# JeanElsner/practical-multi-view

Measured on AMD Instinct MI355X. Metric: VO frames/sec on 1241x376 KITTI mono @400 tracks, bundle=5, higher is better.
Workload: dtype u8/int32 front-end, f64 back-end

## Files before the change

### practical-multi-view_amd/csrc/backend_ba.hip

```cpp
#include "pmv_ctx.h"
#include <algorithm>
#include "backend.h"
#include "pmv_prof.h"
#include <float.h>

namespace pmv {

typedef double v4d __attribute__((ext_vector_type(4)));

constexpr int BA_T = 512;
constexpr int BA_NW = BA_T / 64;


__device__ inline void angle_axis_rotate(const double a[3], const double q[3], double p[3], double dpdw[9], double Rm[9], bool jac) {
    const double theta2 = a[0] * a[0] + a[1] * a[1] + a[2] * a[2];
    if (theta2 > DBL_EPSILON) {
        const double theta = sqrt(theta2);
        const double ct = cos(theta), st = sin(theta), ti = 1.0 / theta;
        const double w[3] = {a[0] * ti, a[1] * ti, a[2] * ti};
        const double wxq[3] = {w[1] * q[2] - w[2] * q[1], w[2] * q[0] - w[0] * q[2], w[0] * q[1] - w[1] * q[0]};
        const double wq = w[0] * q[0] + w[1] * q[1] + w[2] * q[2];
        const double tmp = wq * (1.0 - ct);
#pragma unroll
        for (int i = 0; i < 3; i++) p[i] = q[i] * ct + wxq[i] * st + w[i] * tmp;
// ... 1103 lines not shown
    gmax_p = wave_max_f64(gmax_p);
    if (lane == 0) red[wid] = gmax_p;
    __syncthreads();
    if (tid == 0) part_gmax[sl] = fmax(fmax(red[0], red[1]), fmax(red[2], red[3]));
    const int eb0 = A.pobs_start[p0], eb1 = A.pobs_start[p1];
    for (int e = eb0 + tid; e < eb1; e += BM_T) {
        const int4 rec = A.erec[e];
        if (rec.w == 2) continue;
        const int c = rec.y, pp = rec.z;
        double w[18], y[18];
        bam_obs_wy(A, Jb, e, rec, sEi + (pp - p0) * 9, w, y);
#pragma unroll
        for (int b = 0; b < 3; b++) {
            const int kr = 3 * pp + b - k0;
            if (kr < 0 || kr >= k1 - k0) continue;
#pragma unroll
            for (int a = 0; a < 6; a++) {
                Wl[(size_t)(6 * c + a) * stride + kr] = w[a * 3 + b];
                Yl[(size_t)(6 * c + a) * stride + kr] = y[a * 3 + b];
            }
        }
    }
    __syncthreads();
    const int tc = A.tiles_c;
    if (wid < A.tiles_r * tc) {
        const int ti = wid / tc, tj = wid - ti * tc;
        const double* pa = Yl + (size_t)(ti * 16 + (lane & 15)) * stride + 4 * (lane >> 4);
        const double* pb = Wl + (size_t)(tj * 16 + (lane & 15)) * stride + 4 * (lane >> 4);
        const v4d acc = schur_tile_mfma(pa, pb, (k1 - k0) / 16);
#pragma unroll
        for (int r = 0; r < 4; r++)
            A.Gpart[((size_t)sl * A.gp_rows + ti * 16 + (lane >> 4) + 4 * r) * ldw + tj * 16 + (lane & 15)] = acc[r];
    }
}

__global__ __launch_bounds__(BM_T) void k_bam_pointgemm(BAArgs A, const BAGState* st_in, BAGState* st_out, const double* part4, int nbp,
                                                        int* chol_flag, double* Ublk, double* rhsblk, double* part_gmax) { BACKEND_PRIO();
    extern __shared__ __attribute__((aligned(16))) double dyn[];
    __shared__ BAGState ss;
    __shared__ double ssc[8];
    const int bid = blockIdx.x;
    if (threadIdx.x == 0) {
        ss = *st_in;
        if (!ss.done) bam_decide(ss, part4, nbp);
        if (bid == 0) *st_out = ss;
    }
    __syncthreads();
    if (bid < A.nc) bam_cam_role(A, ss, bid, Ublk, rhsblk, dyn, ssc);
    else bam_slice_role(A, ss, chol_flag, bid - A.nc, part_gmax, dyn);
}

constexpr int BG_W = 4, BG_H = 2;
__device__ inline void bam_gemm_role(const BAArgs& A, const BAGState* st, int bid, double* sacc ) {
    static_assert(BG_W * 4 * 64 <= BM_NW * 4 * 64, "LDS");
    if (st->done) return;
    const int lane = threadIdx.x & 63, wv = threadIdx.x >> 6, krows = A.krows, ldw = A.ldw;
    const int tc = A.tiles_c;
    const int tile = bid / BG_H, half = bid % BG_H;
    const int ti = tile / tc, tj = tile - ti * tc;
    const int kper = A.kper;
    const int k0 = min(krows, (half * BG_W + wv) * kper), k1 = min(krows, k0 + kper);
    const double* pa = A.Yd + (size_t)(ti * 16 + (lane & 15)) * krows + 4 * (lane >> 4) + k0;
    const double* pb = A.Wd + (size_t)(tj * 16 + (lane & 15)) * krows + 4 * (lane >> 4) + k0;
    const v4d acc = schur_tile_mfma(pa, pb, (k1 - k0) / 16);
#pragma unroll
    for (int r = 0; r < 4; r++) sacc[(wv * 4 + r) * 64 + lane] = acc[r];
    __syncthreads();
    if (wv == 0) {
#pragma unroll
        for (int r = 0; r < 4; r++) {
            double g = sacc[r * 64 + lane];
#pragma unroll
            for (int w = 1; w < BG_W; w++) g += sacc[(w * 4 + r) * 64 + lane];
            A.Gpart[((size_t)half * A.gp_rows + ti * 16 + (lane >> 4) + 4 * r) * ldw + tj * 16 + (lane & 15)] = g;
        }
    }
}

__global__ __launch_bounds__(64 * BG_W) void k_bam_gemm(BAArgs A, const BAGState* st) { BACKEND_PRIO();
    __shared__ double swork[BG_W * 4 * 64];
    bam_gemm_role(A, st, blockIdx.x, swork);
}

__device__ inline const BAGState* bam_solve_role(const BAArgs& A, const BAGState* st_in, BAGState* st_out, bool writer,
                                                 const int* __restrict__ chol_flag, const double* __restrict__ part_cost,
                                                 int nbo, const double* __restrict__ part_gmax, int nbp, const double* __restrict__ Ublk,
                                                 const double* __restrict__ rhsblk, double* __restrict__ candrot, double* candrot_l, int gslices) {
    extern __shared__ __attribute__((aligned(16))) double dyn[];
    __shared__ double red[3 * BM_NW];
    __shared__ BAGState ss;
    __shared__ int sfail;
    const int tid = threadIdx.x, lane = tid & 63, wid = tid >> 6;
    const int tx = tid & 15, ty = tid >> 4;
    unsigned long long t_prev = __builtin_readcyclecounter();
#define SSTAMP(k) do { if (A.stamps && writer && tid == 0) { const unsigned long long t_ = __builtin_readcyclecounter(); A.stamps[k] += t_ - t_prev; t_prev = t_; } } while (0)
#define SPUBLISH() do { if (writer && tid == 0) *st_out = ss; } while (0)
    if (tid == 0) { ss = *st_in; sfail = 0; }
    __syncthreads();
    if (ss.done) { SPUBLISH(); return nullptr; }
    const int nc = A.nc, m = 6 * nc, n = m + 3 * A.np;
    double* S = dyn; double* dg = dyn + (size_t)(m + 1) * m;
    const double* x = A.x + (size_t)ss.cur * n;
    if (ss.need_eval) {
        double g = 0, cs = 0;
        for (int i = tid; i < m; i += BM_T) g = fmax(g, fabs(rhsblk[i] / A.scale[i]));
        for (int i = tid; i < nbp; i += BM_T) g = fmax(g, part_gmax[i]);
        for (int i = tid; i < nbo; i += BM_T) cs += part_cost[i];
        cs = wave_sum_f64(cs);
        g = wave_max_f64(g);
        if (lane == 0) { red[BM_NW + wid] = cs; red[2 * BM_NW + wid] = g; }
        __syncthreads();
        if (tid == 0) {
            if (ss.first) {
                const double c = (red[BM_NW] + red[BM_NW + 1]) + (red[BM_NW + 2] + red[BM_NW + 3]);
                ss.x_cost = c;
                ss.initial_cost = c;
            }
            ss.gmax = fmax(fmax(red[2 * BM_NW], red[2 * BM_NW + 1]), fmax(red[2 * BM_NW + 2], red[2 * BM_NW + 3]));
        }
    }
    if (tid == 0) {
        int term = -1;
        if (ss.iter >= ss.max_iterations) term = 0;
        else if (ss.gmax >= 0 && ss.gmax <= 1e-10) term = 2;
        else if (ss.radius < 1e-32) term = 4;
        if (term >= 0) { ss.done = 1; ss.termination = term; }
        ss.step_valid = 0;
    }
    __syncthreads();
    if (ss.done) { SPUBLISH(); return nullptr; }
    SSTAMP(16);
    {
        const double radius = ss.radius;
        const bool reuse = ss.reuse_diag != 0;
        for (int a = ty; a <= m; a += 16) {
            for (int b = tx; b < m && b <= a; b += 16) {
                double v;
                if (a < m) v = (a / 6 == b / 6) ? Ublk[(a / 6) * 36 + (a % 6) * 6 + (b % 6)] : 0.0;
                else v = rhsblk[b];
                const size_t gi = (a < m) ? (size_t)a * A.ldw + b : (size_t)b * A.ldw + m;
                double g;
                if (gslices) {
                    double hsum[BG_H];
#pragma unroll
                    for (int h = 0; h < BG_H; h++) {
#pragma unroll
                        for (int w = 0; w < BG_W; w++) {
                            const int sl = h * BG_W + w;
                            const double v = sl < gslices ? A.Gpart[(size_t)sl * A.gp_rows * A.ldw + gi] : 0.0;
                            hsum[h] = w == 0 ? v : hsum[h] + v;
                        }
                    }
                    g = hsum[0];
#pragma unroll
                    for (int h = 1; h < BG_H; h++) g += hsum[h];
                } else {
                    g = A.Gpart[gi];
#pragma unroll
                    for (int h = 1; h < BG_H; h++) g += A.Gpart[(size_t)h * A.gp_rows * A.ldw + gi];
                }
                if (a == b) {
                    double d2;
                    if (!reuse) { d2 = fmin(fmax(v, 1e-6), 1e32); if (writer) A.diag[a] = d2; }
                    else d2 = A.diag[a];
                    v += d2 / radius;
                }
                S[(size_t)a * m + b] = v - g;
            }
        }
    }
    __syncthreads();
    if (*chol_flag) { SPUBLISH(); return nullptr; }
    SSTAMP(17);
    for (int jb = 0; jb < nc; jb++) {
        const int j0 = 6 * jb;
        if (tid == 0) {
            double a[21];
#pragma unroll
            for (int i = 0; i < 6; i++) {
#pragma unroll
                for (int k = 0; k <= i; k++) a[i * (i + 1) / 2 + k] = S[(size_t)(j0 + i) * m + j0 + k];
            }
            bool ok = true;
            double r[6];
#pragma unroll
            for (int j = 0; j < 6; j++) {
                const double d = a[j * (j + 1) / 2 + j];
                ok = ok && (d > 0.0);
                r[j] = rsqrt_nr(d);
                a[j * (j + 1) / 2 + j] = d * r[j];
#pragma unroll
                for (int i = j + 1; i < 6; i++) a[i * (i + 1) / 2 + j] *= r[j];
#pragma unroll
                for (int i = j + 1; i < 6; i++) {
#pragma unroll
                    for (int k = j + 1; k <= i; k++) a[i * (i + 1) / 2 + k] -= a[i * (i + 1) / 2 + j] * a[k * (k + 1) / 2 + j];
                }
            }
#pragma unroll
            for (int i = 0; i < 6; i++) {
#pragma unroll
                for (int k = 0; k <= i; k++) S[(size_t)(j0 + i) * m + j0 + k] = a[i * (i + 1) / 2 + k];
                dg[j0 + i] = r[i];
            }
            if (!ok) sfail = 1;
        }
        __syncthreads();
        if (sfail) break;
        {
            const int i = j0 + 6 + tid;
            if (i <= m) {
                double v[6], Lb[15], r[6];
#pragma unroll
                for (int k = 0; k < 6; k++) { v[k] = S[(size_t)i * m + j0 + k]; r[k] = dg[j0 + k]; }
#pragma unroll
                for (int q = 1; q < 6; q++) {
#pragma unroll
                    for (int k = 0; k < q; k++) Lb[q * (q - 1) / 2 + k] = S[(size_t)(j0 + q) * m + j0 + k];
                }
#pragma unroll
                for (int q = 0; q < 6; q++) {
                    double t = v[q];
#pragma unroll
                    for (int k = 0; k < q; k++) t -= v[k] * Lb[q * (q - 1) / 2 + k];
                    v[q] = t * r[q];
                }
#pragma unroll
                for (int k = 0; k < 6; k++) S[(size_t)i * m + j0 + k] = v[k];
            }
        }
        __syncthreads();
        {
            const int r0 = j0 + 6;
            const int nr = m - r0;
            const int total = nr * (nr + 1) / 2 + nr;
            for (int e = tid; e < total; e += BM_T) {
                int ii = (int)((sqrtf(8.0f * (float)e + 1.0f) - 1.0f) * 0.5f);
                while ((ii + 1) * (ii + 2) / 2 <= e) ii++;
                while (ii * (ii + 1) / 2 > e) ii--;
                int kk = e - ii * (ii + 1) / 2;
                if (ii >= nr) { ii = nr; kk = e - nr * (nr + 1) / 2; }
                const double* Li = S + (size_t)(r0 + ii) * m + j0;
                const double* Lk = S + (size_t)(r0 + kk) * m + j0;
                double acc = S[(size_t)(r0 + ii) * m + r0 + kk];
#pragma unroll
                for (int t = 0; t < 6; t++) acc -= Li[t] * Lk[t];
                S[(size_t)(r0 + ii) * m + r0 + kk] = acc;
            }
        }
        __syncthreads();
    }
    if (sfail) { SPUBLISH(); return nullptr; }
    SSTAMP(18);
    if (wid == 0) {
        double* ys = S + (size_t)m * m;
        for (int jb = nc - 1; jb >= 0; jb--) {
            const int j0 = 6 * jb;
            double xb[6], Lb[15], r[6];
#pragma unroll
            for (int q = 0; q < 6; q++) { xb[q] = ys[j0 + q]; r[q] = dg[j0 + q]; }
#pragma unroll
            for (int q = 1; q < 6; q++) {
#pragma unroll
                for (int k = 0; k < q; k++) Lb[q * (q - 1) / 2 + k] = S[(size_t)(j0 + q) * m + j0 + k];
            }
#pragma unroll
            for (int q = 5; q >= 0; q--) {
                double t = xb[q];
#pragma unroll
                for (int k = 5; k > q; k--) t -= Lb[k * (k - 1) / 2 + q] * xb[k];
                xb[q] = t * r[q];
            }
            for (int k = lane; k < j0; k += 64) {
                double acc = ys[k];
#pragma unroll
                for (int t = 5; t >= 0; t--) acc -= S[(size_t)(j0 + t) * m + k] * xb[t];
                ys[k] = acc;
            }
            if (lane < 6) {
                double v = xb[0];
#pragma unroll
                for (int t = 1; t < 6; t++) v = (lane == t) ? xb[t] : v;
                ys[j0 + lane] = v;
            }
            WAVE_SYNC();
        }
        for (int k = lane; k < m; k += 64) { const double v = -ys[k]; if (writer) A.step[k] = v; S[k] = v; }
        WAVE_SYNC();
        SSTAMP(19);
        if (lane < nc) {
            double cx[6];
#pragma unroll
            for (int k = 0; k < 6; k++) cx[k] = x[6 * lane + k] + S[6 * lane + k] * A.scale[6 * lane + k];
            CamRot cr;
            cam_rot_setup(cx, cr);
            const double cv[7] = {cr.ct, cr.st, cr.ti, cr.w0, cr.w1, cr.w2, (double)cr.big};
            if (writer) {
                double* o = candrot + 16 * lane;
#pragma unroll
                for (int k = 0; k < 6; k++) o[k] = cx[k];
#pragma unroll
                for (int k = 0; k < 7; k++) o[6 + k] = cv[k];
            }
            if (candrot_l) {
                double* o = candrot_l + 16 * lane;
#pragma unroll
                for (int k = 0; k < 6; k++) o[k] = cx[k];
#pragma unroll
                for (int k = 0; k < 7; k++) o[6 + k] = cv[k];
            }
        }
        if (lane == 0) ss.step_valid = 1;
        SSTAMP(20);
    }
    __syncthreads();
    SPUBLISH();
    return &ss;
#undef SPUBLISH
#undef SSTAMP
}

__device__ inline void bam_backsub_role(const BAArgs& A, const BAGState* st, const double* step_c, const double* candrot,
                                        double* __restrict__ tmp3, double* __restrict__ part4, int bid) {
    __shared__ double red[4 * BM_NW];
    __shared__ double sP[BM_PB * 6];
    if (st->done || !st->step_valid) return;
    const int tid = threadIdx.x;
    unsigned long long t_prev = __builtin_readcyclecounter();
#define BSTAMP(k) do { if (A.stamps && bid == 0 && tid == 0) { const unsigned long long t_ = __builtin_readcyclecounter(); A.stamps[k] += t_ - t_prev; t_prev = t_; } } while (0)
    const int nc = A.nc, m = 6 * nc, n = m + 3 * A.np;
    const int cur = st->cur;
    const double* x = A.x + (size_t)cur * n;
    double* cand = A.x + (size_t)(cur ^ 1) * n;
    const double* Jb = A.J + (size_t)cur * A.nobs * 18;
    const double* resb = A.res + (size_t)cur * A.nobs * 2;
    double* Jn = A.J + (size_t)(cur ^ 1) * A.nobs * 18;
    double* resn = A.res + (size_t)(cur ^ 1) * A.nobs * 2;
    const bool spec = st->iter + 1 < st->max_iterations;
    const int p0 = bid * BM_PB, p1 = min(A.np, p0 + BM_PB);
    const int eb0 = A.pobs_start[p0], eb1 = A.pobs_start[p1];
    double mc = 0, cc = 0, dn2 = 0, xn2 = 0;
    for (int e = eb0 + tid; e < eb1; e += BM_T) {
        const int4 rec = A.erec[e];
        const int i = rec.x, c = rec.y;
        const double* Jr = Jb + (size_t)i * 18;
        double jy0 = 0, jy1 = 0;
#pragma unroll
        for (int a = 0; a < 6; a++) { const double yc = -step_c[6 * c + a]; jy0 += Jr[a] * yc; jy1 += Jr[6 + a] * yc; }
#pragma unroll
        for (int a = 0; a < 3; a++) tmp3[(size_t)e * 3 + a] = Jr[12 + a] * jy0 + Jr[15 + a] * jy1;
    }
    __syncthreads();
    BSTAMP(10);
    const int p = p0 + tid;
    if (tid < BM_PB && p < p1) {
        double t3[3] = {A.gp[(size_t)p * 3], A.gp[(size_t)p * 3 + 1], A.gp[(size_t)p * 3 + 2]};
        for (int e = A.pobs_start[p]; e < A.pobs_start[p + 1]; e++) {
#pragma unroll
            for (int a = 0; a < 3; a++) t3[a] -= tmp3[(size_t)e * 3 + a];
        }
        const double* Ei = A.Einv + (size_t)p * 9;
#pragma unroll
        for (int a = 0; a < 3; a++) {
            const double sp = -(Ei[a * 3] * t3[0] + Ei[a * 3 + 1] * t3[1] + Ei[a * 3 + 2] * t3[2]);
            A.step[m + 3 * p + a] = sp;
            const double d = sp * A.scale[m + 3 * p + a];
            const double xo = x[m + 3 * p + a];
            xn2 += xo * xo;
            const double xp = xo + d;
            cand[m + 3 * p + a] = xp;
            sP[tid * 6 + a] = sp; sP[tid * 6 + 3 + a] = xp;
            dn2 += d * d;
        }
    }
    __syncthreads();
    BSTAMP(11);
    for (int e = eb0 + tid; e < eb1; e += BM_T) {
        const int4 rec = A.erec[e];
        const int i = rec.x, c = rec.y, pl = rec.z - p0;
        const double* Jr = Jb + (size_t)i * 18;
        double sc[6], sp[3], xp[3];
#pragma unroll
        for (int k = 0; k < 6; k++) sc[k] = step_c[6 * c + k];
#pragma unroll
        for (int k = 0; k < 3; k++) { sp[k] = sP[pl * 6 + k]; xp[k] = sP[pl * 6 + 3 + k]; }
#pragma unroll
        for (int rr = 0; rr < 2; rr++) {
            double mr = 0;
#pragma unroll
            for (int k = 0; k < 6; k++) mr += Jr[rr * 6 + k] * sc[k];
#pragma unroll
            for (int k = 0; k < 3; k++) mr += Jr[12 + rr * 3 + k] * sp[k];
            mc -= mr * (resb[2 * i + rr] + mr / 2.0);
        }
        const double* o = candrot + 16 * c;
        CamRot cr;
        cr.ct = o[6]; cr.st = o[7]; cr.ti = o[8]; cr.w0 = o[9]; cr.w1 = o[10]; cr.w2 = o[11]; cr.big = (int)o[12];
        double r[2], rho0, rho1;
        if (spec) {
            double Jc[12], Jp[6];
            projection_residual_pre(cr, o, xp, A.obs[2 * i], A.obs[2 * i + 1], A.K, r, Jc, Jp, true);
            huber_rho(r[0] * r[0] + r[1] * r[1], A.huber, rho0, rho1);
            const double sr = sqrt(rho1);
            resn[2 * i] = r[0] * sr; resn[2 * i + 1] = r[1] * sr;
            const double* scc = A.scale + 6 * c;
            const double* scp = A.scale + 6 * A.nc + 3 * (pl + p0);
            double* Jo = Jn + (size_t)i * 18;
#pragma unroll
            for (int k = 0; k < 12; k++) Jo[k] = Jc[k] * sr * scc[k % 6];
#pragma unroll
            for (int k = 0; k < 6; k++) Jo[12 + k] = Jp[k] * sr * scp[k % 3];
        } else {
            projection_residual_pre(cr, o, xp, A.obs[2 * i], A.obs[2 * i + 1], A.K, r, nullptr, nullptr, false);
            huber_rho(r[0] * r[0] + r[1] * r[1], A.huber, rho0, rho1);
        }
        cc += 0.5 * rho0;
    }
    BSTAMP(12);
    if (bid == 0) {
        for (int i = tid; i < m; i += BM_T) {
            const double d = step_c[i] * A.scale[i];
            cand[i] = x[i] + d;
            dn2 += d * d;
            xn2 += x[i] * x[i];
        }
    }
    mc = wave_sum_f64(mc); cc = wave_sum_f64(cc); dn2 = wave_sum_f64(dn2); xn2 = wave_sum_f64(xn2);
    if ((tid & 63) == 0) { red[tid >> 6] = mc; red[BM_NW + (tid >> 6)] = cc; red[2 * BM_NW + (tid >> 6)] = dn2; red[3 * BM_NW + (tid >> 6)] = xn2; }
    __syncthreads();
    if (tid == 0) {
        part4[bid * 4] = (red[0] + red[1]) + (red[2] + red[3]);
        part4[bid * 4 + 1] = (red[BM_NW] + red[BM_NW + 1]) + (red[BM_NW + 2] + red[BM_NW + 3]);
        part4[bid * 4 + 2] = (red[2 * BM_NW] + red[2 * BM_NW + 1]) + (red[2 * BM_NW + 2] + red[2 * BM_NW + 3]);
        part4[bid * 4 + 3] = (red[3 * BM_NW] + red[3 * BM_NW + 1]) + (red[3 * BM_NW + 2] + red[3 * BM_NW + 3]);
    }
    BSTAMP(13);
#undef BSTAMP
}

__global__ __launch_bounds__(BM_T) void k_bam_solveback(BAArgs A, const BAGState* st_in, BAGState* st_out, const int* chol_flag,
                                                        const double* part_cost, int nbo, const double* part_gmax, int ngm,
                                                        const double* Ublk, const double* rhsblk, double* candrot, double* tmp3,
                                                        double* part4, int gslices) { BACKEND_PRIO();
    extern __shared__ __attribute__((aligned(16))) double dyn[];
    const int m = 6 * A.nc;
    double* candrot_l = dyn + (size_t)(m + 1) * m + m;
    const BAGState* ss = bam_solve_role(A, st_in, st_out, blockIdx.x == 0, chol_flag, part_cost, nbo, part_gmax, ngm, Ublk, rhsblk, candrot, candrot_l, gslices);
    if (!ss) return;
    bam_backsub_role(A, ss, dyn, candrot_l, tmp3, part4, blockIdx.x);
}

__device__ inline void bam_finish_role(const BAArgs& A, const BAGState* __restrict__ st_in, const double* __restrict__ part4, int nbp) {
    __shared__ BAGState ss;
    if (threadIdx.x == 0) {
        ss = *st_in;
        if (!ss.done) bam_decide(ss, part4, nbp);
    }
    __syncthreads();
    const int n = 6 * A.nc + 3 * A.np;
    const double* x = A.x + (size_t)ss.cur * n;
    double* ocams = A.out ? A.out + BA_SUM_SLOTS : A.cams;
    double* opts = A.out ? A.out + BA_SUM_SLOTS + 6 * A.nc : A.pts;
    double* osum = A.out ? A.out : A.summary;
    for (int i = threadIdx.x; i < 6 * A.nc; i += BM_T) ocams[i] = x[i];
    for (int i = threadIdx.x; i < 3 * A.np; i += BM_T) opts[i] = x[6 * A.nc + i];
    if (threadIdx.x == 0) {
        osum[0] = ss.initial_cost; osum[1] = ss.x_cost; osum[2] = ss.iter; osum[3] = ss.successful;
        osum[4] = ss.termination;
    }
    if (A.out && A.done_seq) {
        __threadfence_system();
        __syncthreads();
        if (threadIdx.x == 0) __hip_atomic_store((unsigned*)(A.out + BA_SUM_DONE), A.done_seq, __ATOMIC_RELEASE, __HIP_MEMORY_SCOPE_SYSTEM);
    }
}

__global__ __launch_bounds__(BM_T) void k_bam_finish(BAArgs A, const BAGState* st_in, const double* part4, int nbp) { BACKEND_PRIO();
    bam_finish_role(A, st_in, part4, nbp);
}

hipError_t launch_ba_multi(hipStream_t s, const BAArgs& A, void* d_state, double* d_part) {
    BAGState* sa = (BAGState*)d_state;
    BAGState* sb = (BAGState*)((char*)d_state + 256);
    int* chol_flags = (int*)((char*)d_state + 512);
    static_assert(sizeof(BAGState) <= 256, "BAGState");
    const int nbo = (A.nobs + BM_T - 1) / BM_T, nbp = (A.np + BM_PB - 1) / BM_PB, m = 6 * A.nc;
    double* part_cost = d_part;
    double* part_gmax = part_cost + nbo;
    double* part4 = part_gmax + nbp + 8;
    double* Ublk = part4 + 4 * nbp;
    double* rhsblk = Ublk + 36 * A.nc;
    double* candrot = rhsblk + 6 * A.nc;
    double* tmp3 = candrot + 16 * A.nc;
    const size_t shm = ((size_t)(m + 1) * m + (size_t)m + (size_t)16 * A.nc) * sizeof(double);
    if (A.max_iterations > BA_MAX_ITERATIONS || shm > 150 * 1024) return hipErrorInvalidValue;
    ProfScope ps(K_BA_LM, s);
    const int tiles = A.tiles_r * A.tiles_c;
    const size_t shm_pg = std::max(bam_slice_lds(A.ldw, A.kper), (size_t)BM_WORK * sizeof(double));
    const bool fused = tiles <= BM_NW && A.kslices <= BG_H * BG_W && shm_pg <= 150 * 1024 && bam_slice_points(A.kper) <= BM_T;
    const int clear_blocks = (int)std::min<size_t>(64, ((size_t)A.krows * A.ldw + 4 * BM_T - 1) / (4 * BM_T));
    { ProfScope p_(K_BAM_EVAL0, s);
    hipLaunchKernelGGL(k_bam_eval0, dim3(nbo + clear_blocks), dim3(BM_T), 0, s, A, sa, chol_flags, part_cost, nbo); }
    for (int it = 0; it < A.max_iterations; it++) {
        int* cf = chol_flags + it;
        if (it == 0) {
            ProfScope p_(K_BAM_CAMPOINT, s);
            hipLaunchKernelGGL(k_bam_campoint, dim3(A.nc), dim3(BM_T), 0, s, A, sa, sa, 0, part4, nbp, cf, A.nc, Ublk, rhsblk, part_gmax);
            hipLaunchKernelGGL(k_bam_campoint, dim3(nbp), dim3(BM_T), 0, s, A, sa, sa, 0, part4, nbp, cf, 0, Ublk, rhsblk, part_gmax);
        } else if (fused) {
            ProfScope p_(K_BAM_POINTGEMM, s);
            hipLaunchKernelGGL(k_bam_pointgemm, dim3(A.nc + A.kslices), dim3(BM_T), shm_pg, s, A, sb, sa, part4, nbp, cf, Ublk, rhsblk, part_gmax);
        } else {
            ProfScope p_(K_BAM_CAMPOINT, s);
            hipLaunchKernelGGL(k_bam_campoint, dim3(A.nc + nbp), dim3(BM_T), 0, s, A, sb, sa, 1, part4, nbp, cf, A.nc, Ublk, rhsblk, part_gmax);
        }
        const bool sliced = fused && it > 0;
        if (!sliced) { ProfScope p_(K_BAM_GEMM, s);
        hipLaunchKernelGGL(k_bam_gemm, dim3(tiles * BG_H), dim3(64 * BG_W), 0, s, A, sa); }
        { ProfScope p_(K_BAM_SOLVEBACK, s);
        hipLaunchKernelGGL(k_bam_solveback, dim3(nbp), dim3(BM_T), shm, s, A, sa, sb, cf, part_cost, nbo, part_gmax, sliced ? A.kslices : nbp, Ublk,
                           rhsblk, candrot, tmp3, part4, sliced ? A.kslices : 0); }
    }
    { ProfScope p_(K_BAM_FINISH, s);
    hipLaunchKernelGGL(k_bam_finish, dim3(1), dim3(BM_T), 0, s, A, sb, part4, nbp); }
    return hipGetLastError();
}

void ba_fill_prob(BAProb& P, const BAArgs& A, void* d_state, double* d_part) {
    P.A = A;
    P.st2[0] = d_state; P.st2[1] = (char*)d_state + 256;
    P.chol_flags = (int*)((char*)d_state + 512);
    P.nbo = (A.nobs + BM_T - 1) / BM_T; P.nbp = (A.np + BM_PB - 1) / BM_PB;
    P.part_cost = d_part; P.part_gmax = P.part_cost + P.nbo; P.part4 = P.part_gmax + P.nbp; P.Ublk = P.part4 + 4 * P.nbp;
    P.rhsblk = P.Ublk + 36 * A.nc; P.candrot = P.rhsblk + 6 * A.nc; P.tmp3 = P.candrot + 16 * A.nc;
    P.clear_blocks = (int)std::min<size_t>(64, ((size_t)A.krows * A.ldw + 4 * BM_T - 1) / (4 * BM_T));
    P.tiles = A.tiles_r * A.tiles_c;
}
__global__ __launch_bounds__(BM_T) void k_bamB_eval0(const BAProb* __restrict__ probs) { BACKEND_PRIO();
    const BAProb& P = probs[blockIdx.y];
    const BAArgs A = P.A;
    const int bx = blockIdx.x;
    if (bx < P.nbo) { bam_eval0_role(A, (BAGState*)P.st2[1], P.chol_flags, P.part_cost, bx, P.nbo); return; }
    const int zb = bx - P.nbo, nzb = P.clear_blocks;
    if (zb >= nzb) return;
    const size_t n2 = (size_t)A.krows * A.ldw;
    double2* z = (double2*)A.Yd;
    for (size_t i = (size_t)zb * BM_T + threadIdx.x; i < n2; i += (size_t)nzb * BM_T) z[i] = double2{0.0, 0.0};
}
__global__ __launch_bounds__(BM_T) void k_bamB_campoint(const BAProb* __restrict__ probs, int it, int part) { BACKEND_PRIO();
    __shared__ double swork[BM_WORK];
    const BAProb& P = probs[blockIdx.y];
    const BAArgs A = P.A;
    BAGState* sin = (BAGState*)P.st2[it & 1];
    BAGState* sc = (BAGState*)P.st2[(it + 1) & 1];
    int* cf = P.chol_flags + it;
    const int bx = blockIdx.x;
    if (part == 0) { if (bx >= A.nc) return; bam_campoint_role(A, sc, sc, false, P.part4, P.nbp, cf, A.nc, P.Ublk, P.rhsblk, P.part_gmax, bx, swork); }
    else if (part == 1) { if (bx >= P.nbp) return; bam_campoint_role(A, sc, sc, false, P.part4, P.nbp, cf, 0, P.Ublk, P.rhsblk, P.part_gmax, bx, swork); }
    else { if (bx >= A.nc + P.nbp) return; bam_campoint_role(A, sin, sc, true, P.part4, P.nbp, cf, A.nc, P.Ublk, P.rhsblk, P.part_gmax, bx, swork); }
}
__global__ __launch_bounds__(64 * BG_W) void k_bamB_gemm(const BAProb* __restrict__ probs, int it) { BACKEND_PRIO();
    __shared__ double swork[BG_W * 4 * 64];
    const BAProb& P = probs[blockIdx.y];
    if ((int)blockIdx.x >= P.tiles * BG_H) return;
    const BAArgs A = P.A;
    bam_gemm_role(A, (const BAGState*)P.st2[(it + 1) & 1], blockIdx.x, swork);
}
__global__ __launch_bounds__(BM_T) void k_bamB_solve(const BAProb* __restrict__ probs, int it) { BACKEND_PRIO();
    const BAProb& P = probs[blockIdx.x];
    const BAArgs A = P.A;
    BAGState* st = (BAGState*)P.st2[(it + 1) & 1];
    bam_solve_role(A, st, st, true, P.chol_flags + it, P.part_cost, P.nbo, P.part_gmax, P.nbp, P.Ublk, P.rhsblk, P.candrot, nullptr, 0);
}
__global__ __launch_bounds__(BM_T) void k_bamB_backsub(const BAProb* __restrict__ probs, int it) { BACKEND_PRIO();
    const BAProb& P = probs[blockIdx.y];
    if ((int)blockIdx.x >= P.nbp) return;
    const BAArgs A = P.A;
    bam_backsub_role(A, (const BAGState*)P.st2[(it + 1) & 1], A.step, P.candrot, P.tmp3, P.part4, blockIdx.x);
}
__global__ __launch_bounds__(BM_T) void k_bamB_finish(const BAProb* __restrict__ probs, int max_it) { BACKEND_PRIO();
    const BAProb& P = probs[blockIdx.x];
    const BAArgs A = P.A;
    bam_finish_role(A, (const BAGState*)P.st2[max_it & 1], P.part4, P.nbp);
}
hipError_t launch_ba_multi_batch(hipStream_t s, const BAProb* d_probs, const BABatchDims& D) {
    if (D.n_probs <= 0) return hipSuccess;
    if (!d_probs || D.max_iterations < 1 || D.max_iterations > BA_MAX_ITERATIONS) return hipErrorInvalidValue;
    const size_t shm = ((size_t)(D.max_m + 1) * D.max_m + (size_t)D.max_m) * sizeof(double);
    if (shm > 150 * 1024) return hipErrorInvalidValue;
    const unsigned np = (unsigned)D.n_probs;
    ProfScope ps(K_BA_LM, s);
    hipLaunchKernelGGL(k_bamB_eval0, dim3(D.max_eval_blocks, np), dim3(BM_T), 0, s, d_probs);
    for (int it = 0; it < D.max_iterations; it++) {
        if (it == 0) {
            hipLaunchKernelGGL(k_bamB_campoint, dim3(D.max_nc, np), dim3(BM_T), 0, s, d_probs, it, 0);
            hipLaunchKernelGGL(k_bamB_campoint, dim3(D.max_nbp, np), dim3(BM_T), 0, s, d_probs, it, 1);
        } else
            hipLaunchKernelGGL(k_bamB_campoint, dim3(D.max_nc + D.max_nbp, np), dim3(BM_T), 0, s, d_probs, it, 2);
        hipLaunchKernelGGL(k_bamB_gemm, dim3(D.max_tiles * BG_H, np), dim3(64 * BG_W), 0, s, d_probs, it);
        hipLaunchKernelGGL(k_bamB_solve, dim3(np), dim3(BM_T), shm, s, d_probs, it);
        hipLaunchKernelGGL(k_bamB_backsub, dim3(D.max_nbp, np), dim3(BM_T), 0, s, d_probs, it);
    }
    hipLaunchKernelGGL(k_bamB_finish, dim3(np), dim3(BM_T), 0, s, d_probs, D.max_iterations);
    return hipGetLastError();
}

hipError_t launch_ba_residuals(hipStream_t s, const double* cams, const double* pts, const double* obs, const int* cam_idx,
                               const int* pt_idx, int nobs, const double* K, double* out_r, double* out_J) {
    if (nobs <= 0) return hipSuccess;
    ProfScope ps(K_BA_RESID, s);
    hipLaunchKernelGGL(k_ba_residuals, dim3((nobs + 255) / 256), dim3(256), 0, s, cams, pts, obs, cam_idx, pt_idx, nobs, K, out_r, out_J);
    return hipGetLastError();
}
hipError_t launch_ba_lm_batch(hipStream_t s, const BAArgs* d_args, int n_probs, int max_m) {
    if (!d_args || n_probs < 1 || max_m < 6) return hipErrorInvalidValue;
    const size_t shm = ((size_t)(max_m + 1) * max_m + (size_t)max_m) * sizeof(double);
    ProfScope ps(K_BA_LM, s);
    hipLaunchKernelGGL(k_ba_lm_batch, dim3(n_probs), dim3(BA_T), shm, s, d_args);
    return hipGetLastError();
}
hipError_t launch_ba_lm(hipStream_t s, const BAArgs& A) {
    const int m = 6 * A.nc;
    const size_t shm = ((size_t)(m + 1) * m + (size_t)m) * sizeof(double);
    ProfScope ps(K_BA_LM, s);
    hipLaunchKernelGGL(k_ba_lm, dim3(1), dim3(BA_T), shm, s, A);
    return hipGetLastError();
}

hipError_t backend_prepare_device() {
    hipError_t e = hipFuncSetAttribute((const void*)k_bam_solveback, hipFuncAttributeMaxDynamicSharedMemorySize, 150 * 1024);
    if (e != hipSuccess) return e;
    e = hipFuncSetAttribute((const void*)k_bam_pointgemm, hipFuncAttributeMaxDynamicSharedMemorySize, 150 * 1024);
    if (e != hipSuccess) return e;
    e = hipFuncSetAttribute((const void*)k_bamB_solve, hipFuncAttributeMaxDynamicSharedMemorySize, 150 * 1024);
    if (e != hipSuccess) return e;
    e = hipFuncSetAttribute((const void*)k_ba_lm_batch, hipFuncAttributeMaxDynamicSharedMemorySize, 150 * 1024);
    if (e != hipSuccess) return e;
    return hipFuncSetAttribute((const void*)k_ba_lm, hipFuncAttributeMaxDynamicSharedMemorySize, 150 * 1024);
}

}
```

Baseline: 3777.

## Prefetch backsub inputs during solve and parallelize block Cholesky with wave-level factorization

The fused solve+backsub kernel now prefetches each block's point, edge-record, Jacobian and residual data into registers while the Schur complement is assembled, so the later backsubstitution does not wait on global loads. The 6x6 diagonal Cholesky is done by a whole wave using readlanes, and runs on wave 0 in parallel with the trailing update done by the other waves, which removes one barrier per block. Schur assembly is templated and unrolled 4-way with the loads batched, and tmp3 may be kept in LDS. This raises register pressure and LDS usage, and the index bookkeeping gets more complex.

```diff
diff --git a/practical-multi-view_amd/csrc/backend_ba.hip b/practical-multi-view_amd/csrc/backend_ba.hip
--- a/practical-multi-view_amd/csrc/backend_ba.hip
+++ b/practical-multi-view_amd/csrc/backend_ba.hip
@@ -1209,10 +1209,158 @@
     bam_gemm_role(A, st, blockIdx.x, swork);
 }
 
-__device__ inline const BAGState* bam_solve_role(const BAArgs& A, const BAGState* st_in, BAGState* st_out, bool writer,
+struct BsFront {
+    int eb0, eb1;
+    int ps0, ps1;
+    int4 rec;
+    double J[18], res[2], ob[2], scc[6], scp[3];
+    double gp[3], Ei[9], xs[3], xo[3];
+    double cam_x, cam_s;
+};
+__device__ __forceinline__ void bs_front_point(const BAArgs& A, int cur, int bid, BsFront& F) {
+    const int tid = threadIdx.x, m = 6 * A.nc, n = m + 3 * A.np;
+    const int p0 = bid * BM_PB, p1 = min(A.np, p0 + BM_PB), p = p0 + tid;
+    F.eb0 = A.pobs_start[p0]; F.eb1 = A.pobs_start[p1];
+    const double* x = A.x + (size_t)cur * n;
+    if (bid == 0 && tid < m) { F.cam_x = x[tid]; F.cam_s = A.scale[tid]; }
+    if (tid < BM_PB && p < p1) {
+        F.ps0 = A.pobs_start[p]; F.ps1 = A.pobs_start[p + 1];
+#pragma unroll
+        for (int a = 0; a < 3; a++) { F.gp[a] = A.gp[(size_t)p * 3 + a]; F.xs[a] = A.scale[m + 3 * p + a]; F.xo[a] = x[m + 3 * p + a]; }
+#pragma unroll
+        for (int k = 0; k < 9; k++) F.Ei[k] = A.Einv[(size_t)p * 9 + k];
+    }
+}
+__device__ __forceinline__ void bs_front_record(const BAArgs& A, BsFront& F) {
+    const int e = F.eb0 + (int)threadIdx.x;
+    if (e < F.eb1) F.rec = A.erec[e];
+}
+__device__ __forceinline__ void bs_front_rows(const BAArgs& A, int cur, BsFront& F) {
+    if (F.eb0 + (int)threadIdx.x >= F.eb1) return;
+    const int i = F.rec.x, c = F.rec.y;
+    const double* Jr = A.J + ((size_t)cur * A.nobs + i) * 18;
+    const double* rr = A.res + ((size_t)cur * A.nobs + i) * 2;
+#pragma unroll
+    for (int k = 0; k < 18; k++) F.J[k] = Jr[k];
+#pragma unroll
+    for (int k = 0; k < 2; k++) { F.res[k] = rr[k]; F.ob[k] = A.obs[2 * i + k]; }
+#pragma unroll
+    for (int k = 0; k < 6; k++) F.scc[k] = A.scale[6 * c + k];
+#pragma unroll
+    for (int k = 0; k < 3; k++) F.scp[k] = A.scale[6 * A.nc + 3 * F.rec.z + k];
+}
+
+__device__ __forceinline__ void tri6_rc(int l, int& r, int& c) {
+    r = (l >= 1) + (l >= 3) + (l >= 6) + (l >= 10) + (l >= 15);
+    c = l - r * (r + 1) / 2;
+}
+__device__ __forceinline__ void tri_rc(int e, int& r, int& c) {
+    int ii = (int)((sqrtf(8.0f * (float)e + 1.0f) - 1.0f) * 0.5f);
+    while ((ii + 1) * (ii + 2) / 2 <= e) ii++;
+    while (ii * (ii + 1) / 2 > e) ii--;
+    r = ii; c = e - ii * (ii + 1) / 2;
+}
+__device__ __forceinline__ bool chol6_wave0(double v, double* S, int m, int j0, double* dg, int lane) {
+    double a[21];
+#pragma unroll
+    for (int k = 0; k < 21; k++) a[k] = readlane_f64(v, k);
+    bool ok = true;
+    double r[6];
+#pragma unroll
+    for (int j = 0; j < 6; j++) {
+        const double d = a[j * (j + 1) / 2 + j];
+        ok = ok && (d > 0.0);
+        r[j] = rsqrt_nr(d);
+        a[j * (j + 1) / 2 + j] = d * r[j];
+#pragma unroll
+        for (int i = j + 1; i < 6; i++) a[i * (i + 1) / 2 + j] *= r[j];
+#pragma unroll
+        for (int i = j + 1; i < 6; i++) {
+#pragma unroll
+            for (int k = j + 1; k <= i; k++) a[i * (i + 1) / 2 + k] -= a[i * (i + 1) / 2 + j] * a[k * (k + 1) / 2 + j];
+        }
+    }
+    if (lane == 0) {
+#pragma unroll
+        for (int i = 0; i < 6; i++) {
+#pragma unroll
+            for (int k = 0; k <= i; k++) S[(size_t)(j0 + i) * m + j0 + k] = a[i * (i + 1) / 2 + k];
+            dg[j0 + i] = r[i];
+        }
+    }
+    return ok;
+}
+
+template <bool REUSE, bool SLICED>
+__device__ __forceinline__ void bam_assemble_S(const BAArgs& A, double* S, int m, const double* __restrict__ Ublk, const double* __restrict__ rhsblk,
+                                               int gslices, double radius, bool writer, int tx, int ty) {
+    constexpr int NG = SLICED ? BG_H * BG_W : BG_H;
+    for (int a0 = ty; a0 <= m; a0 += 32) {
+        for (int b0 = tx; b0 < m && b0 <= a0 + 16; b0 += 32) {
+            bool on[4];
+            int ea[4], eb[4];
+            double u[4], rh[4], gpv[4][NG], dv[4];
+#pragma unroll
+            for (int q = 0; q < 4; q++) {
+                const int a = a0 + 16 * (q >> 1), b = b0 + 16 * (q & 1);
+                on[q] = a <= m && b < m && b <= a;
+                ea[q] = on[q] ? a : m; eb[q] = on[q] ? b : 0;
+            }
+#pragma unroll
+            for (int q = 0; q < 4; q++) {
+                const int a = ea[q], b = eb[q];
+                u[q] = Ublk[(a < m && a / 6 == b / 6) ? (a / 6) * 36 + (a % 6) * 6 + (b % 6) : 0];
+                rh[q] = rhsblk[b];
+                const size_t gi = (a < m) ? (size_t)a * A.ldw + b : (size_t)b * A.ldw + m;
+#pragma unroll
+                for (int s = 0; s < NG; s++) gpv[q][s] = A.Gpart[(size_t)(SLICED ? min(s, gslices - 1) : s) * A.gp_rows * A.ldw + gi];
+                dv[q] = REUSE ? A.diag[min(a, m - 1)] : 0.0;
+            }
+#pragma unroll
+            for (int q = 0; q < 4; q++) {
+                if (!on[q]) continue;
+                const int a = ea[q], b = eb[q];
+                double v;
+                if (a < m) v = (a / 6 == b / 6) ? u[q] : 0.0;
+                else v = rh[q];
+                double g;
+                if (SLICED) {
+                    double hsum[BG_H];
+#pragma unroll
+                    for (int h = 0; h < BG_H; h++) {
+#pragma unroll
+                        for (int w = 0; w < BG_W; w++) {
+                            const int sl = h * BG_W + w;
+                            const double gv = sl < gslices ? gpv[q][SLICED ? sl : 0] : 0.0;
+                            hsum[h] = w == 0 ? gv : hsum[h] + gv;
+                        }
+                    }
+                    g = hsum[0];
+#pragma unroll
+                    for (int h = 1; h < BG_H; h++) g += hsum[h];
+                } else {
+                    g = gpv[q][0];
+#pragma unroll
+                    for (int h = 1; h < BG_H; h++) g += gpv[q][h];
+                }
+                if (a == b) {
+                    double d2;
+                    if (!REUSE) { d2 = fmin(fmax(v, 1e-6), 1e32); if (writer) A.diag[a] = d2; }
+                    else d2 = dv[q];
+                    v += d2 / radius;
+                }
+                S[(size_t)a * m + b] = v - g;
+            }
+        }
+    }
+}
+
+template <bool FUSED>
+__device__ __forceinline__ const BAGState* bam_solve_role(const BAArgs& A, const BAGState* st_in, BAGState* st_out, bool writer,
                                                  const int* __restrict__ chol_flag, const double* __restrict__ part_cost,
                                                  int nbo, const double* __restrict__ part_gmax, int nbp, const double* __restrict__ Ublk,
-                                                 const double* __restrict__ rhsblk, double* __restrict__ candrot, double* candrot_l, int gslices) {
+                                                 const double* __restrict__ rhsblk, double* __restrict__ candrot, double* candrot_l, int gslices,
+                                                 BsFront& F, int bid) {
     extern __shared__ __attribute__((aligned(16))) double dyn[];
     __shared__ double red[3 * BM_NW];
     __shared__ BAGState ss;
@@ -1225,14 +1373,28 @@
     if (tid == 0) { ss = *st_in; sfail = 0; }
     __syncthreads();
     if (ss.done) { SPUBLISH(); return nullptr; }
+    SSTAMP(21);
     const int nc = A.nc, m = 6 * nc, n = m + 3 * A.np;
     double* S = dyn; double* dg = dyn + (size_t)(m + 1) * m;
     const double* x = A.x + (size_t)ss.cur * n;
+    const int cflag = *chol_flag;
+    double cam_x[6], cam_s[6];
+    if (tid < nc) {
+#pragma unroll
+        for (int k = 0; k < 6; k++) { cam_x[k] = x[6 * tid + k]; cam_s[k] = A.scale[6 * tid + k]; }
+    }
+    if (FUSED) bs_front_point(A, ss.cur, bid, F);
     if (ss.need_eval) {
+        double q_r = 0, q_s = 1, q_g = 0, q_c = 0;
+        if (tid < m) { q_r = rhsblk[tid]; q_s = A.scale[tid]; }
+        if (tid < nbp) q_g = part_gmax[tid];
+        if (tid < nbo) q_c = part_cost[tid];
         double g = 0, cs = 0;
-        for (int i = tid; i < m; i += BM_T) g = fmax(g, fabs(rhsblk[i] / A.scale[i]));
-        for (int i = tid; i < nbp; i += BM_T) g = fmax(g, part_gmax[i]);
-        for (int i = tid; i < nbo; i += BM_T) cs += part_cost[i];
+        if (tid < m) g = fmax(g, fabs(q_r / q_s));
+        if (tid < nbp) g = fmax(g, q_g);
+        for (int i = tid + BM_T; i < nbp; i += BM_T) g = fmax(g, part_gmax[i]);
+        if (tid < nbo) cs += q_c;
+        for (int i = tid + BM_T; i < nbo; i += BM_T) cs += part_cost[i];
         cs = wave_sum_f64(cs);
         g = wave_max_f64(g);
         if (lane == 0) { red[BM_NW + wid] = cs; red[2 * BM_NW + wid] = g; }
@@ -1257,82 +1419,30 @@
     __syncthreads();
     if (ss.done) { SPUBLISH(); return nullptr; }
     SSTAMP(16);
+    if (FUSED) bs_front_record(A, F);
     {
         const double radius = ss.radius;
-        const bool reuse = ss.reuse_diag != 0;
-        for (int a = ty; a <= m; a += 16) {
-            for (int b = tx; b < m && b <= a; b += 16) {
-                double v;
-                if (a < m) v = (a / 6 == b / 6) ? Ublk[(a / 6) * 36 + (a % 6) * 6 + (b % 6)] : 0.0;
-                else v = rhsblk[b];
-                const size_t gi = (a < m) ? (size_t)a * A.ldw + b : (size_t)b * A.ldw + m;
-                double g;
-                if (gslices) {
-                    double hsum[BG_H];
-#pragma unroll
-                    for (int h = 0; h < BG_H; h++) {
-#pragma unroll
-                        for (int w = 0; w < BG_W; w++) {
-                            const int sl = h * BG_W + w;
-                            const double v = sl < gslices ? A.Gpart[(size_t)sl * A.gp_rows * A.ldw + gi] : 0.0;
-                            hsum[h] = w == 0 ? v : hsum[h] + v;
-                        }
-                    }
-                    g = hsum[0];
-#pragma unroll
-                    for (int h = 1; h < BG_H; h++) g += hsum[h];
-                } else {
-                    g = A.Gpart[gi];
-#pragma unroll
-                    for (int h = 1; h < BG_H; h++) g += A.Gpart[(size_t)h * A.gp_rows * A.ldw + gi];
-                }
-                if (a == b) {
-                    double d2;
-                    if (!reuse) { d2 = fmin(fmax(v, 1e-6), 1e32); if (writer) A.diag[a] = d2; }
-                    else d2 = A.diag[a];
-                    v += d2 / radius;
-                }
-                S[(size_t)a * m + b] = v - g;
-            }
-        }
-    }
-    __syncthreads();
-    if (*chol_flag) { SPUBLISH(); return nullptr; }
+        if (ss.reuse_diag) { if (gslices) bam_assemble_S<true, true>(A, S, m, Ublk, rhsblk, gslices, radius, writer, tx, ty);
+                             else bam_assemble_S<true, false>(A, S, m, Ublk, rhsblk, gslices, radius, writer, tx, ty); }
+        else { if (gslices) bam_assemble_S<false, true>(A, S, m, Ublk, rhsblk, gslices, radius, writer, tx, ty);
+               else bam_assemble_S<false, false>(A, S, m, Ublk, rhsblk, gslices, radius, writer, tx, ty); }
+    }
+    if (FUSED) bs_front_rows(A, ss.cur, F);
+    __syncthreads();
+    if (cflag) { SPUBLISH(); return nullptr; }
     SSTAMP(17);
+    int tl_r, tl_c;
+    tri6_rc(min(lane, 20), tl_r, tl_c);
+    constexpr int TU_T = BM_T - 64;
+    int tu_r = 0, tu_c = 0;
+    if (wid > 0) tri_rc(21 + tid - 64, tu_r, tu_c);
+    if (wid == 0) {
+        const double v = lane < 21 ? S[(size_t)tl_r * m + tl_c] : 0.0;
+        if (!chol6_wave0(v, S, m, 0, dg, lane) && lane == 0) sfail = 1;
+    }
+    __syncthreads();
     for (int jb = 0; jb < nc; jb++) {
         const int j0 = 6 * jb;
-        if (tid == 0) {
-            double a[21];
-#pragma unroll
-            for (int i = 0; i < 6; i++) {
-#pragma unroll
-                for (int k = 0; k <= i; k++) a[i * (i + 1) / 2 + k] = S[(size_t)(j0 + i) * m + j0 + k];
-            }
-            bool ok = true;
-            double r[6];
-#pragma unroll
-            for (int j = 0; j < 6; j++) {
-                const double d = a[j * (j + 1) / 2 + j];
-                ok = ok && (d > 0.0);
-                r[j] = rsqrt_nr(d);
-                a[j * (j + 1) / 2 + j] = d * r[j];
-#pragma unroll
-                for (int i = j + 1; i < 6; i++) a[i * (i + 1) / 2 + j] *= r[j];
-#pragma unroll
-                for (int i = j + 1; i < 6; i++) {
-#pragma unroll
-                    for (int k = j + 1; k <= i; k++) a[i * (i + 1) / 2 + k] -= a[i * (i + 1) / 2 + j] * a[k * (k + 1) / 2 + j];
-                }
-            }
-#pragma unroll
-            for (int i = 0; i < 6; i++) {
-#pragma unroll
-                for (int k = 0; k <= i; k++) S[(size_t)(j0 + i) * m + j0 + k] = a[i * (i + 1) / 2 + k];
-                dg[j0 + i] = r[i];
-            }
-            if (!ok) sfail = 1;
-        }
-        __syncthreads();
         if (sfail) break;
         {
             const int i = j0 + 6 + tid;
@@ -1357,15 +1467,25 @@
             }
         }
         __syncthreads();
-        {
-            const int r0 = j0 + 6;
-            const int nr = m - r0;
-            const int total = nr * (nr + 1) / 2 + nr;
-            for (int e = tid; e < total; e += BM_T) {
-                int ii = (int)((sqrtf(8.0f * (float)e + 1.0f) - 1.0f) * 0.5f);
-                while ((ii + 1) * (ii + 2) / 2 <= e) ii++;
-                while (ii * (ii + 1) / 2 > e) ii--;
-                int kk = e - ii * (ii + 1) / 2;
+        SSTAMP(22);
+        if (jb + 1 == nc) break;
+        const int r0 = j0 + 6;
+        const int nr = m - r0;
+        const int total = nr * (nr + 1) / 2 + nr;
+        if (wid == 0) {
+            double acc = 0.0;
+            if (lane < 21) {
+                const double* Li = S + (size_t)(r0 + tl_r) * m + j0;
+                const double* Lk = S + (size_t)(r0 + tl_c) * m + j0;
+                acc = S[(size_t)(r0 + tl_r) * m + r0 + tl_c];
+#pragma unroll
+                for (int t = 0; t < 6; t++) acc -= Li[t] * Lk[t];
+            }
+            if (!chol6_wave0(acc, S, m, r0, dg, lane) && lane == 0) sfail = 1;
+        } else {
+            int ri = tu_r, ci = tu_c;
+            for (int e = 21 + tid - 64; e < total; e += TU_T) {
+                int ii = ri, kk = ci;
                 if (ii >= nr) { ii = nr; kk = e - nr * (nr + 1) / 2; }
                 const double* Li = S + (size_t)(r0 + ii) * m + j0;
                 const double* Lk = S + (size_t)(r0 + kk) * m + j0;
@@ -1373,9 +1493,12 @@
 #pragma unroll
                 for (int t = 0; t < 6; t++) acc -= Li[t] * Lk[t];
                 S[(size_t)(r0 + ii) * m + r0 + kk] = acc;
+                ci += TU_T;
+                while (ci > ri) { ci -= ri + 1; ri++; }
             }
         }
         __syncthreads();
+        SSTAMP(23);
     }
     if (sfail) { SPUBLISH(); return nullptr; }
     SSTAMP(18);
@@ -1418,7 +1541,7 @@
         if (lane < nc) {
             double cx[6];
 #pragma unroll
-            for (int k = 0; k < 6; k++) cx[k] = x[6 * lane + k] + S[6 * lane + k] * A.scale[6 * lane + k];
+            for (int k = 0; k < 6; k++) cx[k] = cam_x[k] + S[6 * lane + k] * cam_s[k];
             CamRot cr;
             cam_rot_setup(cx, cr);
             const double cv[7] = {cr.ct, cr.st, cr.ti, cr.w0, cr.w1, cr.w2, (double)cr.big};
@@ -1447,8 +1570,9 @@
 #undef SSTAMP
 }
 
-__device__ inline void bam_backsub_role(const BAArgs& A, const BAGState* st, const double* step_c, const double* candrot,
-                                        double* __restrict__ tmp3, double* __restrict__ part4, int bid) {
+__device__ __forceinline__ void bam_backsub_role(const BAArgs& A, const BAGState* st, const double* step_c, const double* candrot,
+                                                 double* __restrict__ tmp3, double* __restrict__ part4, int bid, const BsFront& F,
+                                                 double* tmp3_l, int tmp3_rows) {
     __shared__ double red[4 * BM_NW];
     __shared__ double sP[BM_PB * 6];
     if (st->done || !st->step_valid) return;
@@ -1457,7 +1581,6 @@
 #define BSTAMP(k) do { if (A.stamps && bid == 0 && tid == 0) { const unsigned long long t_ = __builtin_readcyclecounter(); A.stamps[k] += t_ - t_prev; t_prev = t_; } } while (0)
     const int nc = A.nc, m = 6 * nc, n = m + 3 * A.np;
     const int cur = st->cur;
-    const double* x = A.x + (size_t)cur * n;
     double* cand = A.x + (size_t)(cur ^ 1) * n;
     const double* Jb = A.J + (size_t)cur * A.nobs * 18;
     const double* resb = A.res + (size_t)cur * A.nobs * 2;
@@ -1465,34 +1588,56 @@
     double* resn = A.res + (size_t)(cur ^ 1) * A.nobs * 2;
     const bool spec = st->iter + 1 < st->max_iterations;
     const int p0 = bid * BM_PB, p1 = min(A.np, p0 + BM_PB);
-    const int eb0 = A.pobs_start[p0], eb1 = A.pobs_start[p1];
+    const int eb0 = F.eb0, eb1 = F.eb1;
+    const bool t3_lds = eb1 - eb0 <= tmp3_rows;
+    if (A.stamps && bid == 0 && tid == 0) { A.stamps[24] += 1; A.stamps[25] += t3_lds ? 1 : 0; }
     double mc = 0, cc = 0, dn2 = 0, xn2 = 0;
     for (int e = eb0 + tid; e < eb1; e += BM_T) {
-        const int4 rec = A.erec[e];
+        const bool first = e == eb0 + tid;
+        const int4 rec = first ? F.rec : A.erec[e];
         const int i = rec.x, c = rec.y;
-        const double* Jr = Jb + (size_t)i * 18;
+        double Jr[18];
+        if (first) {
+#pragma unroll
+            for (int k = 0; k < 18; k++) Jr[k] = F.J[k];
+        } else {
+#pragma unroll
+            for (int k = 0; k < 18; k++) Jr[k] = Jb[(size_t)i * 18 + k];
+        }
         double jy0 = 0, jy1 = 0;
 #pragma unroll
         for (int a = 0; a < 6; a++) { const double yc = -step_c[6 * c + a]; jy0 += Jr[a] * yc; jy1 += Jr[6 + a] * yc; }
-#pragma unroll
-        for (int a = 0; a < 3; a++) tmp3[(size_t)e * 3 + a] = Jr[12 + a] * jy0 + Jr[15 + a] * jy1;
+        if (t3_lds) {
+#pragma unroll
+            for (int a = 0; a < 3; a++) tmp3_l[(e - eb0) * 3 + a] = Jr[12 + a] * jy0 + Jr[15 + a] * jy1;
+        } else {
+#pragma unroll
+            for (int a = 0; a < 3; a++) tmp3[(size_t)e * 3 + a] = Jr[12 + a] * jy0 + Jr[15 + a] * jy1;
+        }
     }
     __syncthreads();
     BSTAMP(10);
     const int p = p0 + tid;
     if (tid < BM_PB && p < p1) {
-        double t3[3] = {A.gp[(size_t)p * 3], A.gp[(size_t)p * 3 + 1], A.gp[(size_t)p * 3 + 2]};
-        for (int e = A.pobs_start[p]; e < A.pobs_start[p + 1]; e++) {
-#pragma unroll
-            for (int a = 0; a < 3; a++) t3[a] -= tmp3[(size_t)e * 3 + a];
-        }
-        const double* Ei = A.Einv + (size_t)p * 9;
+        double t3[3] = {F.gp[0], F.gp[1], F.gp[2]};
+        if (t3_lds) {
+            for (int e = F.ps0; e < F.ps1; e++) {
+#pragma unroll
+                for (int a = 0; a < 3; a++) t3[a] -= tmp3_l[(e - eb0) * 3 + a];
+            }
+        } else {
+            for (int e = F.ps0; e < F.ps1; e++) {
+#pragma unroll
+                for (int a = 0; a < 3; a++) t3[a] -= tmp3[(size_t)e * 3 + a];
+            }
+        }
+        const double* Ei = F.Ei;
 #pragma unroll
         for (int a = 0; a < 3; a++) {
             const double sp = -(Ei[a * 3] * t3[0] + Ei[a * 3 + 1] * t3[1] + Ei[a * 3 + 2] * t3[2]);
             A.step[m + 3 * p + a] = sp;
-            const double d = sp * A.scale[m + 3 * p + a];
-            const double xo = x[m + 3 * p + a];
+            const double d = sp * F.xs[a];
+            const double xo = F.xo[a];
             xn2 += xo * xo;
             const double xp = xo + d;
             cand[m + 3 * p + a] = xp;
@@ -1503,9 +1648,29 @@
     __syncthreads();
     BSTAMP(11);
     for (int e = eb0 + tid; e < eb1; e += BM_T) {
-        const int4 rec = A.erec[e];
+        const bool first = e == eb0 + tid;
+        const int4 rec = first ? F.rec : A.erec[e];
         const int i = rec.x, c = rec.y, pl = rec.z - p0;
-        const double* Jr = Jb + (size_t)i * 18;
+        double Jr[18], rs[2], ob[2], scc[6], scp[3];
+        if (first) {
+#pragma unroll
+            for (int k = 0; k < 18; k++) Jr[k] = F.J[k];
+#pragma unroll
+            for (int k = 0; k < 2; k++) { rs[k] = F.res[k]; ob[k] = F.ob[k]; }
+#pragma unroll
+            for (int k = 0; k < 6; k++) scc[k] = F.scc[k];
+#pragma unroll
+            for (int k = 0; k < 3; k++) scp[k] = F.scp[k];
+        } else {
+#pragma unroll
+            for (int k = 0; k < 18; k++) Jr[k] = Jb[(size_t)i * 18 + k];
+#pragma unroll
+            for (int k = 0; k < 2; k++) { rs[k] = resb[2 * i + k]; ob[k] = A.obs[2 * i + k]; }
+#pragma unroll
+            for (int k = 0; k < 6; k++) scc[k] = A.scale[6 * c + k];
+#pragma unroll
+            for (int k = 0; k < 3; k++) scp[k] = A.scale[6 * A.nc + 3 * rec.z + k];
+        }
         double sc[6], sp[3], xp[3];
 #pragma unroll
         for (int k = 0; k < 6; k++) sc[k] = step_c[6 * c + k];
@@ -1518,7 +1683,7 @@
             for (int k = 0; k < 6; k++) mr += Jr[rr * 6 + k] * sc[k];
 #pragma unroll
             for (int k = 0; k < 3; k++) mr += Jr[12 + rr * 3 + k] * sp[k];
-            mc -= mr * (resb[2 * i + rr] + mr / 2.0);
+            mc -= mr * (rs[rr] + mr / 2.0);
         }
         const double* o = candrot + 16 * c;
         CamRot cr;
@@ -1526,30 +1691,29 @@
         double r[2], rho0, rho1;
         if (spec) {
             double Jc[12], Jp[6];
-            projection_residual_pre(cr, o, xp, A.obs[2 * i], A.obs[2 * i + 1], A.K, r, Jc, Jp, true);
+            projection_residual_pre(cr, o, xp, ob[0], ob[1], A.K, r, Jc, Jp, true);
             huber_rho(r[0] * r[0] + r[1] * r[1], A.huber, rho0, rho1);
             const double sr = sqrt(rho1);
             resn[2 * i] = r[0] * sr; resn[2 * i + 1] = r[1] * sr;
-            const double* scc = A.scale + 6 * c;
-            const double* scp = A.scale + 6 * A.nc + 3 * (pl + p0);
             double* Jo = Jn + (size_t)i * 18;
 #pragma unroll
             for (int k = 0; k < 12; k++) Jo[k] = Jc[k] * sr * scc[k % 6];
 #pragma unroll
             for (int k = 0; k < 6; k++) Jo[12 + k] = Jp[k] * sr * scp[k % 3];
         } else {
-            projection_residual_pre(cr, o, xp, A.obs[2 * i], A.obs[2 * i + 1], A.K, r, nullptr, nullptr, false);
+            projection_residual_pre(cr, o, xp, ob[0], ob[1], A.K, r, nullptr, nullptr, false);
             huber_rho(r[0] * r[0] + r[1] * r[1], A.huber, rho0, rho1);
         }
         cc += 0.5 * rho0;
     }
     BSTAMP(12);
     if (bid == 0) {
-        for (int i = tid; i < m; i += BM_T) {
-            const double d = step_c[i] * A.scale[i];
-            cand[i] = x[i] + d;
+        if (tid < m) {
+            const int i = tid;
+            const double d = step_c[i] * F.cam_s;
+            cand[i] = F.cam_x + d;
             dn2 += d * d;
-            xn2 += x[i] * x[i];
+            xn2 += F.cam_x * F.cam_x;
         }
     }
     mc = wave_sum_f64(mc); cc = wave_sum_f64(cc); dn2 = wave_sum_f64(dn2); xn2 = wave_sum_f64(xn2);
@@ -1568,13 +1732,15 @@
 __global__ __launch_bounds__(BM_T) void k_bam_solveback(BAArgs A, const BAGState* st_in, BAGState* st_out, const int* chol_flag,
                                                         const double* part_cost, int nbo, const double* part_gmax, int ngm,
                                                         const double* Ublk, const double* rhsblk, double* candrot, double* tmp3,
-                                                        double* part4, int gslices) { BACKEND_PRIO();
+                                                        double* part4, int gslices, int tmp3_rows) { BACKEND_PRIO();
     extern __shared__ __attribute__((aligned(16))) double dyn[];
     const int m = 6 * A.nc;
     double* candrot_l = dyn + (size_t)(m + 1) * m + m;
-    const BAGState* ss = bam_solve_role(A, st_in, st_out, blockIdx.x == 0, chol_flag, part_cost, nbo, part_gmax, ngm, Ublk, rhsblk, candrot, candrot_l, gslices);
+    BsFront F = {};
+    const BAGState* ss = bam_solve_role<true>(A, st_in, st_out, blockIdx.x == 0, chol_flag, part_cost, nbo, part_gmax, ngm, Ublk, rhsblk, candrot, candrot_l,
+                                              gslices, F, blockIdx.x);
     if (!ss) return;
-    bam_backsub_role(A, ss, dyn, candrot_l, tmp3, part4, blockIdx.x);
+    bam_backsub_role(A, ss, dyn, candrot_l, tmp3, part4, blockIdx.x, F, candrot_l + 16 * A.nc, tmp3_rows);
 }
 
 __device__ inline void bam_finish_role(const BAArgs& A, const BAGState* __restrict__ st_in, const double* __restrict__ part4, int nbp) {
@@ -1606,6 +1772,9 @@
     bam_finish_role(A, st_in, part4, nbp);
 }
 
+static int bam_tmp3_lds_rows(size_t shm_solve, int nobs) {
+    return (int)std::min<size_t>((size_t)std::max(nobs, 0), (150 * 1024 - shm_solve) / (3 * sizeof(double)));
+}
 hipError_t launch_ba_multi(hipStream_t s, const BAArgs& A, void* d_state, double* d_part) {
     BAGState* sa = (BAGState*)d_state;
     BAGState* sb = (BAGState*)((char*)d_state + 256);
@@ -1619,8 +1788,10 @@
     double* rhsblk = Ublk + 36 * A.nc;
     double* candrot = rhsblk + 6 * A.nc;
     double* tmp3 = candrot + 16 * A.nc;
-    const size_t shm = ((size_t)(m + 1) * m + (size_t)m + (size_t)16 * A.nc) * sizeof(double);
-    if (A.max_iterations > BA_MAX_ITERATIONS || shm > 150 * 1024) return hipErrorInvalidValue;
+    const size_t shm_s = ((size_t)(m + 1) * m + (size_t)m + (size_t)16 * A.nc) * sizeof(double);
+    if (A.max_iterations > BA_MAX_ITERATIONS || shm_s > 150 * 1024) return hipErrorInvalidValue;
+    const int tmp3_rows = bam_tmp3_lds_rows(shm_s, A.nobs);
+    const size_t shm = shm_s + (size_t)tmp3_rows * 3 * sizeof(double);
     ProfScope ps(K_BA_LM, s);
     const int tiles = A.tiles_r * A.tiles_c;
     const size_t shm_pg = std::max(bam_slice_lds(A.ldw, A.kper), (size_t)BM_WORK * sizeof(double));
@@ -1646,7 +1817,7 @@
         hipLaunchKernelGGL(k_bam_gemm, dim3(tiles * BG_H), dim3(64 * BG_W), 0, s, A, sa); }
         { ProfScope p_(K_BAM_SOLVEBACK, s);
         hipLaunchKernelGGL(k_bam_solveback, dim3(nbp), dim3(BM_T), shm, s, A, sa, sb, cf, part_cost, nbo, part_gmax, sliced ? A.kslices : nbp, Ublk,
-                           rhsblk, candrot, tmp3, part4, sliced ? A.kslices : 0); }
+                           rhsblk, candrot, tmp3, part4, sliced ? A.kslices : 0, tmp3_rows); }
     }
     { ProfScope p_(K_BAM_FINISH, s);
     hipLaunchKernelGGL(k_bam_finish, dim3(1), dim3(BM_T), 0, s, A, sb, part4, nbp); }
@@ -1697,13 +1868,20 @@
     const BAProb& P = probs[blockIdx.x];
     const BAArgs A = P.A;
     BAGState* st = (BAGState*)P.st2[(it + 1) & 1];
-    bam_solve_role(A, st, st, true, P.chol_flags + it, P.part_cost, P.nbo, P.part_gmax, P.nbp, P.Ublk, P.rhsblk, P.candrot, nullptr, 0);
+    BsFront F;
+    bam_solve_role<false>(A, st, st, true, P.chol_flags + it, P.part_cost, P.nbo, P.part_gmax, P.nbp, P.Ublk, P.rhsblk, P.candrot, nullptr, 0, F, 0);
 }
 __global__ __launch_bounds__(BM_T) void k_bamB_backsub(const BAProb* __restrict__ probs, int it) { BACKEND_PRIO();
     const BAProb& P = probs[blockIdx.y];
     if ((int)blockIdx.x >= P.nbp) return;
     const BAArgs A = P.A;
-    bam_backsub_role(A, (const BAGState*)P.st2[(it + 1) & 1], A.step, P.candrot, P.tmp3, P.part4, blockIdx.x);
+    const BAGState* st = (const BAGState*)P.st2[(it + 1) & 1];
+    if (st->done || !st->step_valid) return;
+    BsFront F = {};
+    bs_front_point(A, st->cur, blockIdx.x, F);
+    bs_front_record(A, F);
+    bs_front_rows(A, st->cur, F);
+    bam_backsub_role(A, st, A.step, P.candrot, P.tmp3, P.part4, blockIdx.x, F, nullptr, -1);
 }
 __global__ __launch_bounds__(BM_T) void k_bamB_finish(const BAProb* __restrict__ probs, int max_it) { BACKEND_PRIO();
     const BAProb& P = probs[blockIdx.x];
```

Result: faster. 3977, median of 6 (+5.3%).
